# sikoba/babble

Measured on AMD Instinct MI355X. Metric: ECDSA event verifies/sec, higher is better.
Workload: dtype u32; 1 GPU; C2: VerifyBatch of 1M signed Events per GPU (64 creators, 1x64-B tx, ~446-B bodies); per-key tables rebuilt every step; events_per_gpu=1000000, creators=64, parallelism=single, batches_in_flight=2

## Files before the change

### babble_amd/csrc/point.h

```cpp
#pragma once
#include "field.h"

struct gej {
  fe X, Y, Z;
};

DEV void gej_double(gej &r, const gej &a) {
  fe A, B, C, D, E, F, t;
  fe_sqr(A, a.X);
  fe_sqr(B, a.Y);
  fe_sqr(C, B);
  fe_add(t, a.X, B);
  fe_sqr(t, t);
  fe_sub(t, t, A);
  fe_sub(t, t, C);
  fe_dbl(D, t);
  fe_dbl(E, A);
  fe_add(E, E, A);
  fe_sqr(F, E);
  fe Z3;
  fe_mul(Z3, a.Y, a.Z);
  fe_dbl(r.Z, Z3);
  fe_dbl(t, D);
  fe_sub(r.X, F, t);
  fe_sub(t, D, r.X);
  fe_mul(r.Y, E, t);
  fe_dbl(t, C);
  fe_dbl(t, t);
  fe_dbl(t, t);
  fe_sub(r.Y, r.Y, t);
}

DEV void gej_double_lat(gej &r, const gej &a) {
#if defined(__HIP_DEVICE_COMPILE__)
  fe A, B, YZ, C, t, E, F, D;
  fe_sqr_sqr_mul_zip_asm(A, a.X, B, a.Y, YZ, a.Y, a.Z);
  fe_add(t, a.X, B);
  fe_dbl(E, A);
  fe_add(E, E, A);
  fe_sqr_sqr_sqr_zip_asm(C, B, t, t, F, E);
  fe_sub(t, t, A);
  fe_sub(t, t, C);
  fe_dbl(D, t);
  fe_dbl(r.Z, YZ);
  fe_dbl(t, D);
  fe_sub(r.X, F, t);
  fe_sub(t, D, r.X);
  fe_mul(r.Y, E, t);
  fe_dbl(t, C);
  fe_dbl(t, t);
  fe_dbl(t, t);
  fe_sub(r.Y, r.Y, t);
#else
  gej_double(r, a);
#endif
}

DEV void gej_add_ge(gej &r, bool &inf, const fe &x2, const fe &y2) {
  if (inf) {
    r.X = x2;
    r.Y = y2;
    fe_set(r.Z, 1);
    inf = false;
    return;
  }
  fe Z1Z1, U2, S2, H, R, t;
  fe_sqr(Z1Z1, r.Z);
  fe_mul(U2, x2, Z1Z1);
  fe_mul(t, r.Z, Z1Z1);
  fe_mul(S2, y2, t);
  fe_sub(H, U2, r.X);
  fe_sub(R, S2, r.Y);
  if (fe_is_zero(H)) {
    if (fe_is_zero(R)) {
      gej d;
      gej_double(d, r);
      r = d;
    } else {
      inf = true;
    }
    return;
  }
  fe HH, HHH, V;
  fe_sqr(HH, H);
  fe_mul(HHH, H, HH);
  fe_mul(V, r.X, HH);
  fe_mul(r.Z, r.Z, H);
  fe_sqr(t, R);
  fe_sub(t, t, HHH);
  fe_sub(t, t, V);
  fe_sub(r.X, t, V);
  fe_sub(t, V, r.X);
  fe_mul(t, R, t);
  fe_mul(HHH, r.Y, HHH);
  fe_sub(r.Y, t, HHH);
}

DEV void gej_add_ge_lat(gej &r, bool &inf, const fe &x2, const fe &y2) {
#if defined(__HIP_DEVICE_COMPILE__)
  if (inf) {
    r.X = x2;
    r.Y = y2;
    fe_set(r.Z, 1);
    inf = false;
    return;
  }
  fe Z1Z1, U2, S2, H, R, t, HH, HHH, V, Z3, RR;
  fe_sqr(Z1Z1, r.Z);
  fe_mul_mul_zip_asm(U2, x2, Z1Z1, t, r.Z, Z1Z1);
  fe_sub(H, U2, r.X);
  fe_mul_sqr_zip_asm(S2, y2, t, HH, H);
  fe_sub(R, S2, r.Y);
  if (fe_is_zero(H)) {
    if (fe_is_zero(R)) {
      gej d;
      gej_double_lat(d, r);
      r = d;
    } else {
      inf = true;
    }
    return;
  }
  fe_mul_mul_mul_sqr_zip_asm(HHH, H, HH, V, r.X, HH, Z3, r.Z, H, RR, R);
  r.Z = Z3;
  fe_sub(t, RR, HHH);
  fe_sub(t, t, V);
  fe_sub(r.X, t, V);
  fe_sub(t, V, r.X);
  fe_mul_mul_zip_asm(t, R, t, HHH, r.Y, HHH);
  fe_sub(r.Y, t, HHH);
#else
  gej_add_ge(r, inf, x2, y2);
#endif
}

template <bool LAT>
DEV void gej_add_ge_sel(gej &r, bool &inf, const fe &x2, const fe &y2) {
  if (LAT) gej_add_ge_lat(r, inf, x2, y2);
  else gej_add_ge(r, inf, x2, y2);
}
template <bool LAT>
DEV void gej_double_sel(gej &r, const gej &a) {
  if (LAT) gej_double_lat(r, a);
  else gej_double(r, a);
}

DEV void gej_add(gej &r, bool &rinf, const gej &b, bool binf) {
  if (binf) return;
  if (rinf) {
    r = b;
    rinf = false;
    return;
  }
  fe Z1Z1, Z2Z2, U1, U2, S1, S2, H, I, J, rr, V, t;
  fe_sqr(Z1Z1, r.Z);
  fe_sqr(Z2Z2, b.Z);
  fe_mul(U1, r.X, Z2Z2);
  fe_mul(U2, b.X, Z1Z1);
  fe_mul(t, b.Z, Z2Z2);
  fe_mul(S1, r.Y, t);
  fe_mul(t, r.Z, Z1Z1);
  fe_mul(S2, b.Y, t);
  fe_sub(H, U2, U1);
  fe_sub(rr, S2, S1);
  if (fe_is_zero(H)) {
    if (fe_is_zero(rr)) {
      gej d;
      gej_double(d, r);
      r = d;
    } else {
      rinf = true;
    }
    return;
  }
  fe_dbl(I, H);
  fe_sqr(I, I);
  fe_mul(J, H, I);
  fe_dbl(rr, rr);
  fe_mul(V, U1, I);
  fe_add(t, r.Z, b.Z);
  fe_sqr(t, t);
  fe_sub(t, t, Z1Z1);
  fe_sub(t, t, Z2Z2);
  fe_mul(r.Z, t, H);
  fe_sqr(t, rr);
  fe_sub(t, t, J);
  fe_sub(t, t, V);
  fe_sub(r.X, t, V);
  fe_sub(t, V, r.X);
  fe_mul(t, rr, t);
  fe_mul(J, S1, J);
  fe_dbl(J, J);
  fe_sub(r.Y, t, J);
}

struct gexz {
  fe X, Y, ZZ, ZZZ;
};

DEV void gexz_double(gexz &r, const gexz &a) {
  fe U, V, W, S, M, t;
  fe_dbl(U, a.Y);
  fe_sqr(V, U);
  fe_mul(W, U, V);
  fe_mul(S, a.X, V);
  fe_sqr(M, a.X);
  fe_dbl(t, M);
  fe_add(M, M, t);
  fe_sqr(t, M);
  fe_dbl(r.X, S);
  fe_sub(r.X, t, r.X);
  fe_sub(t, S, r.X);
  fe_mul(t, M, t);
  fe_mul(U, W, a.Y);
  fe_sub(r.Y, t, U);
  fe_mul(r.ZZ, V, a.ZZ);
  fe_mul(r.ZZZ, W, a.ZZZ);
}

DEV void gexz_set_ge(gexz &r, const fe &x, const fe &y) {
  r.X = x;
  r.Y = y;
  fe_set(r.ZZ, 1);
  fe_set(r.ZZZ, 1);
}

DEV void gexz_add_ge(gexz &r, bool &inf, const fe &x2, const fe &y2) {
  if (inf) {
    gexz_set_ge(r, x2, y2);
    inf = false;
    return;
  }
  fe P, R, PP, PPP, Q, t;
  fe_mul(P, x2, r.ZZ);
  fe_sub(P, P, r.X);
  fe_mul(R, y2, r.ZZZ);
  fe_sub(R, R, r.Y);
  if (fe_is_zero(P)) {
    if (fe_is_zero(R)) {
      gexz d;
      gexz_double(d, r);
      r = d;
    } else {
      inf = true;
    }
    return;
  }
  fe_sqr(PP, P);
  fe_mul(PPP, P, PP);
  fe_mul(Q, r.X, PP);
  fe_mul(r.ZZ, r.ZZ, PP);
  fe_sqr(t, R);
  fe_sub(t, t, PPP);
  fe_sub(t, t, Q);
  fe_sub(r.X, t, Q);
  fe_sub(t, Q, r.X);
  fe_mul(t, R, t);
  fe_mul(r.ZZZ, r.ZZZ, PPP);
  fe_mul(PPP, r.Y, PPP);
  fe_sub(r.Y, t, PPP);
}

DEV void gexz_add_ge_lat(gexz &r, bool &inf, const fe &x2, const fe &y2) {
#if defined(__HIP_DEVICE_COMPILE__)
  if (inf) {
    gexz_set_ge(r, x2, y2);
    inf = false;
    return;
  }
  fe P, R, PP, RR, PPP, Q, ZZ3, t, u;
  fe_mul_mul_zip_asm(P, x2, r.ZZ, R, y2, r.ZZZ);
  fe_sub(P, P, r.X);
  fe_sub(R, R, r.Y);
  if (fe_is_zero(P)) {
    if (fe_is_zero(R)) {
      gexz d;
      gexz_double(d, r);
      r = d;
    } else {
      inf = true;
    }
    return;
  }
  fe_sqr_sqr_zip_asm(PP, P, RR, R);
  fe_mul_mul_mul_zip_asm(PPP, P, PP, Q, r.X, PP, ZZ3, r.ZZ, PP);
  r.ZZ = ZZ3;
  fe_sub(t, RR, PPP);
  fe_sub(t, t, Q);
  fe_sub(r.X, t, Q);
  fe_sub(t, Q, r.X);
  fe_mul_mul_mul_zip_asm(t, R, t, u, r.Y, PPP, ZZ3, r.ZZZ, PPP);
  r.ZZZ = ZZ3;
  fe_sub(r.Y, t, u);
#else
  gexz_add_ge(r, inf, x2, y2);
#endif
}

DEV void gexz_add(gexz &r, bool &rinf, const gexz &b, bool binf) {
  if (binf) return;
  if (rinf) {
    r = b;
    rinf = false;
    return;
  }
  fe U1, U2, S1, S2, P, R, PP, PPP, Q, t;
  fe_mul(U1, r.X, b.ZZ);
  fe_mul(U2, b.X, r.ZZ);
  fe_mul(S1, r.Y, b.ZZZ);
  fe_mul(S2, b.Y, r.ZZZ);
  fe_sub(P, U2, U1);
  fe_sub(R, S2, S1);
  if (fe_is_zero(P)) {
    if (fe_is_zero(R)) {
      gexz d;
      gexz_double(d, r);
      r = d;
    } else {
      rinf = true;
    }
    return;
  }
  fe_sqr(PP, P);
  fe_mul(PPP, P, PP);
  fe_mul(Q, U1, PP);
  fe_sqr(t, R);
  fe_sub(t, t, PPP);
  fe_sub(t, t, Q);
  fe_sub(r.X, t, Q);
  fe_sub(t, Q, r.X);
  fe_mul(t, R, t);
  fe_mul(S1, S1, PPP);
  fe_sub(r.Y, t, S1);
  fe_mul(r.ZZ, r.ZZ, b.ZZ);
  fe_mul(r.ZZ, r.ZZ, PP);
  fe_mul(r.ZZZ, r.ZZZ, b.ZZZ);
  fe_mul(r.ZZZ, r.ZZZ, PPP);
}

DEV void gexz_add_lat(gexz &r, bool &rinf, const gexz &b, bool binf) {
#if defined(__HIP_DEVICE_COMPILE__)
  if (binf) return;
  if (rinf) {
    r = b;
    rinf = false;
    return;
  }
  fe U1, U2, S1, S2, Z12, W12, P, R, PP, RR, PPP, Q, t, u;
  fe_mul_mul_mul_zip_asm(U1, r.X, b.ZZ, U2, b.X, r.ZZ, S1, r.Y, b.ZZZ);
  fe_mul_mul_mul_zip_asm(S2, b.Y, r.ZZZ, Z12, r.ZZ, b.ZZ, W12, r.ZZZ, b.ZZZ);
  fe_sub(P, U2, U1);
  fe_sub(R, S2, S1);
  if (fe_is_zero(P)) {
    if (fe_is_zero(R)) {
      gexz d;
      gexz_double(d, r);
      r = d;
    } else {
      rinf = true;
    }
    return;
  }
  fe_sqr_sqr_zip_asm(PP, P, RR, R);
  fe_mul_mul_mul_zip_asm(PPP, P, PP, Q, U1, PP, r.ZZ, Z12, PP);
  fe_sub(t, RR, PPP);
  fe_sub(t, t, Q);
  fe_sub(r.X, t, Q);
  fe_sub(t, Q, r.X);
  fe_mul_mul_mul_zip_asm(t, R, t, u, S1, PPP, r.ZZZ, W12, PPP);
  fe_sub(r.Y, t, u);
#else
  gexz_add(r, rinf, b, binf);
#endif
}

DEV void gexz_sum_ge_lat(gexz &r, bool &rinf, const fe &x1, const fe &y1, bool i1, const fe &x2, const fe &y2,
                         bool i2) {
  rinf = i1 && i2;
  if (i1 || i2) {
    if (!rinf) gexz_set_ge(r, i1 ? x2 : x1, i1 ? y2 : y1);
    return;
  }
  fe P, R;
  fe_sub(P, x2, x1);
  fe_sub(R, y2, y1);
  if (fe_is_zero(P)) {
    if (fe_is_zero(R)) {
      gexz a;
      gexz_set_ge(a, x1, y1);
      gexz_double(r, a);
    } else {
      rinf = true;
    }
    return;
  }
#if defined(__HIP_DEVICE_COMPILE__)
  fe PP, RR, PPP, Q, t, u;
  fe_sqr_sqr_zip_asm(PP, P, RR, R);
  fe_mul_mul_zip_asm(PPP, P, PP, Q, x1, PP);
  fe_sub(t, RR, PPP);
  fe_sub(t, t, Q);
  fe_sub(r.X, t, Q);
  fe_sub(t, Q, r.X);
  fe_mul_mul_zip_asm(t, R, t, u, y1, PPP);
  fe_sub(r.Y, t, u);
  r.ZZ = PP;
  r.ZZZ = PPP;
#else
  gexz_set_ge(r, x1, y1);
  gexz_add_ge(r, rinf, x2, y2);
#endif
}

DEV void gexz_from_gej(gexz &r, const gej &a) {
  r.X = a.X;
  r.Y = a.Y;
  fe_sqr(r.ZZ, a.Z);
  fe_mul(r.ZZZ, r.ZZ, a.Z);
}

template <bool LAT>
DEV void pt_add_ge(gexz &r, bool &inf, const fe &x2, const fe &y2) {
  if (LAT) gexz_add_ge_lat(r, inf, x2, y2);
  else gexz_add_ge(r, inf, x2, y2);
}

template <bool LAT>
DEV void gexz_add_ge_aff(gexz &r, bool &inf, const fe &x2, const fe &y2) {
  fe P, R, PP, RR, PPP, Q, t, u, v;
  fe_sub(P, x2, r.X);
  fe_sub(R, y2, r.Y);
  if (fe_is_zero(P)) {
    if (fe_is_zero(R)) {
      gexz d;
      gexz_double(d, r);
      r = d;
    } else {
      inf = true;
    }
    return;
  }
#if defined(__HIP_DEVICE_COMPILE__)
  if (LAT) {
    fe_sqr_sqr_zip_asm(PP, P, RR, R);
    fe_mul_mul_zip_asm(PPP, P, PP, Q, r.X, PP);
  } else
#endif
  {
    fe_sqr(PP, P);
    fe_sqr(RR, R);
    fe_mul(PPP, P, PP);
    fe_mul(Q, r.X, PP);
  }
  fe_sub(t, RR, PPP);
  fe_sub(t, t, Q);
  fe_sub(t, t, Q);
  fe_sub(u, Q, t);
  r.X = t;
  r.ZZ = PP;
  r.ZZZ = PPP;
#if defined(__HIP_DEVICE_COMPILE__)
  if (LAT) {
    fe_mul_mul_zip_asm(t, R, u, v, r.Y, PPP);
  } else
#endif
  {
    fe_mul(t, R, u);
    fe_mul(v, r.Y, PPP);
  }
  fe_sub(r.Y, t, v);
}

template <bool LAT>
DEV void pt_add_ge_step(gexz &r, bool &inf, const fe &x2, const fe &y2, bool take) {
  if (take) pt_add_ge<LAT>(r, inf, x2, y2);
}
template <bool LAT>
DEV void pt_add_ge_step(gej &r, bool &inf, const fe &x2, const fe &y2, bool take) {
  if (take) gej_add_ge_sel<LAT>(r, inf, x2, y2);
}
template <bool LAT>
DEV void pt_add_ge(gej &r, bool &inf, const fe &x2, const fe &y2) {
  gej_add_ge_sel<LAT>(r, inf, x2, y2);
}
```

### babble_amd/csrc/verify_core.h

```cpp
#pragma once
#include <type_traits>
#include <stdint.h>

#include "../../include/babbleverify.h"
#include "geometry.h"
#include "coop.h"
#include "point.h"
#include "sha256.h"

#define KS_OK 0
#define KS_EMPTY 1
#define KS_BAD 2

static constexpr uint32_t P_MINUS_N[8] = {0x2FC9BAEEu, 0x402DA172u, 0x50B75FC4u, 0x45512319u,
                                          0x00000001u, 0u, 0u, 0u};

DEV void fe_load_be(fe &r, const uint8_t *b) {
#pragma unroll
  for (int i = 0; i < 8; i++) {
    const uint8_t *q = b + 4 * (7 - i);
    r.v[i] = ((uint32_t)q[0] << 24) | ((uint32_t)q[1] << 16) | ((uint32_t)q[2] << 8) | q[3];
  }
}
DEV void fe_load_be_words(fe &r, const uint32_t *w) {
#pragma unroll
  for (int i = 0; i < 8; i++) r.v[i] = bswap32(w[7 - i]);
}
DEV void sc_load_be_words(sc &r, const uint32_t *w) {
#pragma unroll
  for (int i = 0; i < 8; i++) r.v[i] = bswap32(w[7 - i]);
}
DEV void fe_store(uint32_t *p, const fe &a) {
#pragma unroll
  for (int i = 0; i < 8; i++) p[i] = a.v[i];
}
DEV void fe_load(fe &a, const uint32_t *p) {
#pragma unroll
  for (int i = 0; i < 8; i++) a.v[i] = p[i];
}
DEV void fe_load4(fe &a, const uint32_t *p) {
#if defined(__HIP_DEVICE_COMPILE__)
  typedef const __attribute__((address_space(1))) uint4 *gptr;
  const gptr q = (gptr)p;
#else
  const uint4 *q = (const uint4 *)p;
#endif
  uint4 l = q[0], h = q[1];
  a.v[0] = l.x; a.v[1] = l.y; a.v[2] = l.z; a.v[3] = l.w;
  a.v[4] = h.x; a.v[5] = h.y; a.v[6] = h.z; a.v[7] = h.w;
}
DEV void store16(uint32_t *p, const uint32_t *v) {
  uint4 *q = (uint4 *)p;
#pragma unroll
  for (int c = 0; c < 4; c++) q[c] = make_uint4(v[4 * c], v[4 * c + 1], v[4 * c + 2], v[4 * c + 3]);
}
DEV bool u256_lt(const uint32_t *a, const uint32_t *b) {
#pragma unroll
  for (int i = 7; i >= 0; i--) {
    if (a[i] != b[i]) return a[i] < b[i];
  }
  return false;
}
DEV bool u256_is_zero(const uint32_t *a) {
  uint32_t x = 0;
#pragma unroll
  for (int i = 0; i < 8; i++) x |= a[i];
  return x == 0;
}

DEV void sha256_one(uint64_t m, const uint8_t *bytes, const uint64_t *off, uint32_t *digest_words) {
  const uint64_t o = off[m];
  const uint64_t len = off[m + 1] - o;
  uint32_t h[8];
  sha256_msg(h, bytes, o, len);
  uint32_t be[8];
#pragma unroll
  for (int i = 0; i < 8; i++) be[i] = bswap32(h[i]);
  uint4 *dst = (uint4 *)(digest_words + 8 * m);
  dst[0] = make_uint4(be[0], be[1], be[2], be[3]);
  dst[1] = make_uint4(be[4], be[5], be[6], be[7]);
}

DEV void key_decode_point(const uint8_t *kbytes, uint64_t o, uint64_t len, uint8_t &st, fe &x, fe &y) {
  st = KS_BAD;
  fe_set(x, 0);
  fe_set(y, 0);
  if (len == 0) {
    st = KS_EMPTY;
  } else if (len == 65 && kbytes[o] == 4) {
#if defined(__HIP_DEVICE_COMPILE__)
    const uint32_t *w = (const uint32_t *)(kbytes + (o & ~(uint64_t)3));
    const uint32_t sh = (uint32_t)(o & 3);
    uint32_t d[18];
#pragma unroll
    for (int i = 0; i < 18; i++) d[i] = w[i];
#pragma unroll
    for (int i = 0; i < 8; i++) {
      const uint32_t bx = 1 + 4 * (7 - i) + sh, by = 33 + 4 * (7 - i) + sh;
      x.v[i] = bswap32(alignbyte(d[bx / 4 + 1], d[bx / 4], bx % 4));
      y.v[i] = bswap32(alignbyte(d[by / 4 + 1], d[by / 4], by % 4));
    }
#else
    fe_load_be(x, kbytes + o + 1);
    fe_load_be(y, kbytes + o + 33);
#endif
    if (!fe_ge_p(x) && !fe_ge_p(y)) {
      fe y2, x3, seven;
      fe_sqr(y2, y);
      fe_sqr(x3, x);
      fe_mul(x3, x3, x);
      fe_set(seven, 7);
      fe_add(x3, x3, seven);
      if (fe_eq(y2, x3)) st = KS_OK;
    }
  }
}

DEV void key_decode_one(uint32_t k, const uint8_t *kbytes, const uint64_t *koff, uint8_t *kstatus, uint32_t *kxy) {
  uint8_t st;
  fe x, y;
  key_decode_point(kbytes, koff[k], koff[k + 1] - koff[k], st, x, y);
  kstatus[k] = st;
  fe_store(kxy + 16 * k, x);
  fe_store(kxy + 16 * k + 8, y);
}

template <bool LAT = false>
DEV void table_bases_one(uint32_t b, const uint32_t *bxy, uint32_t *bases_jac, int w, int nwin) {
  gej P;
  fe_load(P.X, bxy + 16 * b);
  fe_load(P.Y, bxy + 16 * b + 8);
  fe_set(P.Z, 1);
  uint32_t *out = bases_jac + (uint64_t)b * nwin * 24;
  for (int j = 0; j < nwin; j++) {
    fe_store(out + 24 * j, P.X);
    fe_store(out + 24 * j + 8, P.Y);
    fe_store(out + 24 * j + 16, P.Z);
    if (j + 1 < nwin) {
      for (int k = 0; k < w; k++) gej_double_sel<LAT>(P, P);
    }
  }
}

#if defined(__HIPCC__)
__device__ __forceinline__ void coop_bases_one(uint32_t b, const uint32_t *bxy, uint32_t *bases_jac, int w, int nwin) {
  const uint32_t k = coop::pos(), lane = __lane_id();
  uint32_t X = k < 8 ? bxy[16 * (uint64_t)b + k] : 0u, Y = k < 8 ? bxy[16 * (uint64_t)b + 8 + k] : 0u;
  uint32_t Z = k == 0 ? 1u : 0u;
  uint32_t *out = bases_jac + (uint64_t)b * nwin * 24;
  for (int j = 0; j < nwin; j++) {
    if (lane < 8) {
      out[24 * j + lane] = X;
      out[24 * j + 8 + lane] = Y;
      out[24 * j + 16 + lane] = Z;
    }
    if (j + 1 < nwin)
      for (int i = 0; i < w; i++) coop::dbl(X, Y, Z);
  }
}
#endif

template <bool LAT = false>
DEV void table_point(gej &R, bool &inf, fe &Z, const fe &bx, const fe &by, uint32_t d, int bits) {
  inf = true;
  fe_set(R.X, 0);
  fe_set(R.Y, 0);
  fe_set(R.Z, 0);
  for (int bit = bits - 1; bit >= 0; bit--) {
    if (!inf) gej_double_sel<LAT>(R, R);
    if ((d >> bit) & 1) gej_add_ge_sel<LAT>(R, inf, bx, by);
  }
  if (inf) fe_set(Z, 1);
  else Z = R.Z;
}

DEV void table_store(uint32_t *entry, uint32_t *phi, uint32_t d, const gej &R, bool inf, const fe &zi) {
  fe zi2, zi3, x, y;
  fe_sqr(zi2, zi);
  fe_mul(zi3, zi2, zi);
  fe_mul(x, R.X, zi2);
  fe_mul(y, R.Y, zi3);
  fe_canon(x);
  fe_canon(y);
  if (d == 0 || inf) {
    fe_set(x, 0);
    fe_set(y, 0);
  }
  uint32_t v[16];
#pragma unroll
  for (int i = 0; i < 8; i++) {
    v[i] = x.v[i];
    v[8 + i] = y.v[i];
  }
  store16(entry, v);
  if (phi) {
    fe beta, bx;
    fe_load(beta, FE_BETA);
    fe_mul(bx, x, beta);
    fe_canon(bx);
#pragma unroll
    for (int i = 0; i < 8; i++) v[i] = bx.v[i];
    store16(phi, v);
  }
}

DEV int pair_kind(uint32_t lo, uint32_t hi) { return (lo ? 1 : 0) | (hi ? 2 : 0); }

DEV uint32_t k12_digit(uint32_t d, uint32_t ent) { return d ? d : ent; }

DEV void pair_load(const uint32_t *s_lo, const uint32_t *s_hi, uint32_t lo, uint32_t hi, fe &x1, fe &y1, fe &x2,
                   fe &y2) {
  fe_load(x1, s_lo + BV_ENTRY_U32 * lo);
  fe_load(y1, s_lo + BV_ENTRY_U32 * lo + 8);
  fe_load(x2, s_hi + BV_ENTRY_U32 * hi);
  fe_load(y2, s_hi + BV_ENTRY_U32 * hi + 8);
}

DEV void pair_denominator(fe &H, int kind, const fe &x1, const fe &x2) {
  if (kind == 3) fe_sub(H, x2, x1);
  else fe_set(H, 1);
}

DEV void pair_store(uint32_t *entry, uint32_t *phi, int kind, const fe &x1, const fe &y1, const fe &x2, const fe &y2,
                    const fe &Hinv) {
  fe x, y;
  if (kind == 3) {
    fe lam, t;
    fe_sub(t, y2, y1);
    fe_mul(lam, t, Hinv);
    fe_sqr(x, lam);
    fe_sub(x, x, x1);
    fe_sub(x, x, x2);
    fe_sub(t, x1, x);
    fe_mul(y, lam, t);
    fe_sub(y, y, y1);
  } else if (kind == 1) {
    x = x1;
    y = y1;
  } else {
    x = x2;
    y = y2;
  }
  fe_canon(x);
  fe_canon(y);
  uint32_t v[16];
#pragma unroll
  for (int i = 0; i < 8; i++) {
    v[i] = x.v[i];
    v[8 + i] = y.v[i];
  }
  store16(entry, v);
  if (!phi) return;
  fe beta, bx;
  fe_load(beta, FE_BETA);
  fe_mul(bx, x, beta);
  fe_canon(bx);
#pragma unroll
  for (int i = 0; i < 8; i++) v[i] = bx.v[i];
  store16(phi, v);
}

DEV void sc_sqrn(sc &a, int n) {
#pragma unroll 1
  for (int i = 0; i < n; i++) sc_mont(a, a, a);
}

DEV void sc_inverse(sc &r, const sc &x) {
  sc x2, x3, x5, x7, x9, x11, x13, x15;
  sc_mont(x2, x, x);
  sc_mont(x3, x2, x);
  sc_mont(x5, x3, x2);
  sc_mont(x7, x5, x2);
  sc_mont(x9, x7, x2);
  sc_mont(x11, x9, x2);
  sc_mont(x13, x11, x2);
  sc_mont(x15, x13, x2);
  sc a2 = x3, a4, a8, a16, a32, a64, t;
  a4 = a2; sc_sqrn(a4, 2); sc_mont(a4, a4, a2);
  a8 = a4; sc_sqrn(a8, 4); sc_mont(a8, a8, a4);
  a16 = a8; sc_sqrn(a16, 8); sc_mont(a16, a16, a8);
  a32 = a16; sc_sqrn(a32, 16); sc_mont(a32, a32, a16);
  a64 = a32; sc_sqrn(a64, 32); sc_mont(a64, a64, a32);
  t = a64;
  sc_sqrn(t, 32); sc_mont(t, t, a32);
  sc_sqrn(t, 16); sc_mont(t, t, a16);
  sc_sqrn(t, 8); sc_mont(t, t, a8);
  sc_sqrn(t, 4); sc_mont(t, t, a4);
  sc_sqrn(t, 2); sc_mont(t, t, a2);
  sc_sqrn(t, 1); sc_mont(t, t, x);
  sc_sqrn(t, 1);
#define SQM(n, m) sc_sqrn(t, n); sc_mont(t, t, m);
  SQM(4, x11) SQM(3, x5) SQM(4, x5) SQM(4, x7) SQM(5, x13) SQM(2, x3) SQM(5, x7) SQM(6, x13)
  SQM(5, x11) SQM(4, x13) SQM(3, x) SQM(6, x5) SQM(10, x7) SQM(4, x7) SQM(5, x15) SQM(4, x15)
  SQM(5, x9) SQM(6, x11) SQM(4, x13) SQM(5, x3) SQM(6, x13) SQM(10, x13) SQM(4, x9) SQM(9, x9)
  SQM(4, x15) SQM(1, x)
#undef SQM
  r = t;
}

DEV bool s_usable(const uint8_t *pre, uint64_t i, const sc &s) {
  return (pre == nullptr || pre[i] == 0) && !u256_is_zero(s.v) && u256_lt(s.v, SC_N);
}

DEV void sinv_thread(uint64_t t, uint64_t T, uint64_t n_items, uint32_t M, const uint32_t *s_be, const uint8_t *pre,
                     uint32_t *w_out) {
  sc R1, one;
  sc_load_const(R1, SC_R1);
#pragma unroll
  for (int k = 0; k < 8; k++) one.v[k] = k == 0 ? 1u : 0u;
  sc acc = R1;
  for (uint32_t m = 0; m < M; m++) {
    const uint64_t i = t + (uint64_t)m * T;
    if (i >= n_items) break;
    sc s;
    sc_load_be_words(s, s_be + 8 * i);
    if (!s_usable(pre, i, s)) s = one;
    uint4 *q = (uint4 *)(w_out + 8 * i);
    q[0] = make_uint4(acc.v[0], acc.v[1], acc.v[2], acc.v[3]);
    q[1] = make_uint4(acc.v[4], acc.v[5], acc.v[6], acc.v[7]);
    sc_mont(acc, acc, s);
  }
  sc inv;
  sc_inverse_var(inv, acc);
  sc_mont(inv, inv, one);
  for (int m = (int)M - 1; m >= 0; m--) {
    const uint64_t i = t + (uint64_t)m * T;
    if (i >= n_items) continue;
    sc s, pfx, w;
    sc_load_be_words(s, s_be + 8 * i);
    if (!s_usable(pre, i, s)) s = one;
    uint4 *q = (uint4 *)(w_out + 8 * i);
    const uint4 a = q[0], b = q[1];
    pfx.v[0] = a.x; pfx.v[1] = a.y; pfx.v[2] = a.z; pfx.v[3] = a.w;
    pfx.v[4] = b.x; pfx.v[5] = b.y; pfx.v[6] = b.z; pfx.v[7] = b.w;
    sc_mont(w, inv, pfx);
    sc_mont(inv, inv, s);
    q[0] = make_uint4(w.v[0], w.v[1], w.v[2], w.v[3]);
    q[1] = make_uint4(w.v[4], w.v[5], w.v[6], w.v[7]);
  }
}

DEV void item_scalars(uint64_t i, const uint32_t *r_be, const uint32_t *item_msg, const uint32_t *digest_words,
                      const uint32_t *w_in, uint32_t u1[8], uint32_t k1[4], uint32_t k2[4], uint32_t &signs) {
  sc w, e, r, a, b;
  const uint4 *q = (const uint4 *)(w_in + 8 * i);
  const uint4 x = q[0], y = q[1];
  w.v[0] = x.x; w.v[1] = x.y; w.v[2] = x.z; w.v[3] = x.w;
  w.v[4] = y.x; w.v[5] = y.y; w.v[6] = y.z; w.v[7] = y.w;
  sc_load_be_words(e, digest_words + 8 * (uint64_t)item_msg[i]);
  sc_load_be_words(r, r_be + 8 * i);
  sc_mont(a, e, w);
  sc_mont(b, r, w);
#pragma unroll
  for (int k = 0; k < 8; k++) u1[k] = a.v[k];
  glv_split(k1, k2, signs, b);
}

#define BV_DEFERRED 0xFE

DEV uint8_t classify(uint8_t pre, uint8_t ks, const fe &r, const fe &s) {
  if (pre & BV_PRE_PARTS_BAD) return BV_REJECT_ERR;
  if (ks == KS_EMPTY) return BV_REF_PANIC;
  uint32_t rc = pre & 3u, scl = (pre >> 2) & 3u;
  if (rc == BV_SC_OK) rc = u256_is_zero(r.v) ? BV_SC_NONPOS : (u256_lt(r.v, SC_N) ? BV_SC_OK : BV_SC_GE_N);
  if (scl == BV_SC_OK) scl = u256_is_zero(s.v) ? BV_SC_NONPOS : (u256_lt(s.v, SC_N) ? BV_SC_OK : BV_SC_GE_N);
  if (rc == BV_SC_NIL) return BV_REF_PANIC;
  if (rc == BV_SC_NONPOS) return BV_REJECT;
  if (scl == BV_SC_NIL) return BV_REF_PANIC;
  if (scl == BV_SC_NONPOS) return BV_REJECT;
  if (rc == BV_SC_GE_N || scl == BV_SC_GE_N) return BV_REJECT;
  if (ks != KS_OK) return BV_REF_PANIC;
  return 0xFF;
}

DEV uint8_t classify_item(uint64_t i, const uint32_t *item_key, const uint32_t *r_be, const uint32_t *s_be,
                          const uint8_t *pre, const uint8_t *kstatus, fe &r) {
  fe s;
  fe_load_be_words(r, r_be + 8 * i);
  fe_load_be_words(s, s_be + 8 * i);
  return classify(pre ? pre[i] : 0, kstatus[item_key[i]], r, s);
}

DEV bool final_check(const gej &R, bool inf, const fe &r) {
  if (inf) return false;
  fe z2, t;
  fe_sqr(z2, R.Z);
  fe_mul(t, r, z2);
  if (fe_eq(t, R.X)) return true;
  if (u256_lt(r.v, P_MINUS_N)) {
    fe rn;
    uint32_t c = 0;
#pragma unroll
    for (int i = 0; i < 8; i++) rn.v[i] = addc32(r.v[i], SC_N[i], c);
    fe_mul(t, rn, z2);
    if (fe_eq(t, R.X)) return true;
  }
  return false;
}

DEV bool final_check(const gexz &R, bool inf, const fe &r) {
  if (inf) return false;
  fe t;
  fe_mul(t, r, R.ZZ);
  if (fe_eq(t, R.X)) return true;
  if (u256_lt(r.v, P_MINUS_N)) {
    fe rn;
    uint32_t c = 0;
#pragma unroll
    for (int i = 0; i < 8; i++) rn.v[i] = addc32(r.v[i], SC_N[i], c);
    fe_mul(t, rn, R.ZZ);
    if (fe_eq(t, R.X)) return true;
  }
  return false;
}

template <int W, int NWIN, bool LAT = false, class PT = gej, bool FROM_INF = false>
DEV void g_table_add(PT &R, bool &inf, const uint32_t *tab, uint32_t u[8]) {
  constexpr uint32_t ENT = 1u << (W - 1);
  static_assert(W * NWIN >= 257 && W < 32, "signed G windows must absorb the last carry");
  uint32_t carry = 0;
  for (int j = 0; j < NWIN; j++) {
    uint32_t d = (u[0] & ((1u << W) - 1u)) + carry;
#pragma unroll
    for (int c = 0; c < 7; c++) u[c] = (u[c] >> W) | (u[c + 1] << (32 - W));
    u[7] >>= W;
    carry = d > ENT ? 1u : 0u;
    const bool dneg = carry != 0;
    if (dneg) d = (1u << W) - d;
    const uint32_t *e = tab + ((uint64_t)j * ENT + d) * BV_ENTRY_U32;
    fe x, y;
    fe_load4(x, e);
    fe_load4(y, e + 8);
    fe_cneg_canon(y, dneg);
    if constexpr (FROM_INF) {
      if (j == 1 && !inf) {
        if (d != 0) gexz_add_ge_aff<LAT>(R, inf, x, y);
        continue;
      }
    }
    pt_add_ge_step<LAT>(R, inf, x, y, d != 0);
  }
}

DEV void load_k(uint32_t k1[4], uint32_t k2[4], uint32_t &signs, const uint32_t *u12, uint64_t i) {
  const uint4 *q = (const uint4 *)(u12 + (uint64_t)BV_U_STRIDE * i);
  uint4 a = q[0], b = q[1], c = q[2];
  k1[0] = a.x; k1[1] = a.y; k1[2] = a.z; k1[3] = a.w;
  k2[0] = b.x; k2[1] = b.y; k2[2] = b.z; k2[3] = b.w;
  signs = c.x;
}

#define RG_WORDS 33
DEV void rg_store(uint32_t *rg, uint64_t n, uint64_t i, const gexz &R, bool inf) {
#pragma unroll
  for (int k = 0; k < 8; k++) {
    rg[(uint64_t)k * n + i] = R.X.v[k];
    rg[(uint64_t)(8 + k) * n + i] = R.Y.v[k];
    rg[(uint64_t)(16 + k) * n + i] = R.ZZ.v[k];
    rg[(uint64_t)(24 + k) * n + i] = R.ZZZ.v[k];
  }
  rg[(uint64_t)32 * n + i] = inf ? 1u : 0u;
}
DEV void rg_load(const uint32_t *rg, uint64_t n, uint64_t i, gexz &R, bool &inf) {
#pragma unroll
  for (int k = 0; k < 8; k++) {
    R.X.v[k] = rg[(uint64_t)k * n + i];
    R.Y.v[k] = rg[(uint64_t)(8 + k) * n + i];
    R.ZZ.v[k] = rg[(uint64_t)(16 + k) * n + i];
    R.ZZZ.v[k] = rg[(uint64_t)(24 + k) * n + i];
  }
  inf = rg[(uint64_t)32 * n + i] != 0;
}

DEV void glv_split_item(uint64_t i, const uint32_t *r_be, const uint32_t *w_in, uint32_t *u12) {
  sc w, r, b;
  const uint4 *q = (const uint4 *)(w_in + 8 * i);
  const uint4 x = q[0], y = q[1];
  w.v[0] = x.x; w.v[1] = x.y; w.v[2] = x.z; w.v[3] = x.w;
  w.v[4] = y.x; w.v[5] = y.y; w.v[6] = y.z; w.v[7] = y.w;
  sc_load_be_words(r, r_be + 8 * i);
  sc_mont(b, r, w);
  uint32_t k1[4], k2[4], signs;
  glv_split(k1, k2, signs, b);
  uint4 *o = (uint4 *)(u12 + (uint64_t)BV_U_STRIDE * i);
  o[0] = make_uint4(k1[0], k1[1], k1[2], k1[3]);
  o[1] = make_uint4(k2[0], k2[1], k2[2], k2[3]);
  o[2] = make_uint4(signs, 0u, 0u, 0u);
}

template <bool LAT = false, bool SPLIT = false>
DEV void verify_item_g(uint64_t i, uint64_t n, const uint32_t *item_key, const uint32_t *r_be, const uint32_t *s_be,
                       const uint8_t *pre, const uint8_t *kstatus, const uint32_t *item_msg,
                       const uint32_t *digest_words, const uint32_t *w_in, uint32_t *u12, const uint32_t *g_table,
                       uint32_t *rg) {
  fe r;
  if (classify_item(i, item_key, r_be, s_be, pre, kstatus, r) != 0xFF) return;
  uint32_t u[8];
  if (SPLIT) {
    sc w, e, a;
    const uint4 *q = (const uint4 *)(w_in + 8 * i);
    const uint4 x = q[0], y = q[1];
    w.v[0] = x.x; w.v[1] = x.y; w.v[2] = x.z; w.v[3] = x.w;
    w.v[4] = y.x; w.v[5] = y.y; w.v[6] = y.z; w.v[7] = y.w;
    sc_load_be_words(e, digest_words + 8 * (uint64_t)item_msg[i]);
    sc_mont(a, e, w);
#pragma unroll
    for (int k = 0; k < 8; k++) u[k] = a.v[k];
  } else {
    uint32_t k1[4], k2[4], signs;
    item_scalars(i, r_be, item_msg, digest_words, w_in, u, k1, k2, signs);
    uint4 *q = (uint4 *)(u12 + (uint64_t)BV_U_STRIDE * i);
    q[0] = make_uint4(k1[0], k1[1], k1[2], k1[3]);
    q[1] = make_uint4(k2[0], k2[1], k2[2], k2[3]);
    q[2] = make_uint4(signs, 0u, 0u, 0u);
  }
  gexz R;
  bool inf = true;
  fe_set(R.X, 0);
  fe_set(R.Y, 0);
  fe_set(R.ZZ, 0);
  fe_set(R.ZZZ, 0);
  g_table_add<BV_GW, BV_GNWIN, LAT, gexz, true>(R, inf, g_table, u);
  rg_store(rg, n, i, R, inf);
}

template <int W, int NWIN, bool SIGNED, bool LAT = false, class PT = gexz>
DEV void key_table_add(PT &R, bool &inf, const uint32_t *tab, uint32_t k[4], bool neg, bool phi = false,
                       bool from_inf = false) {
  constexpr uint32_t ENT = SIGNED ? (1u << (W - 1)) : (1u << W);
  static_assert(!SIGNED || W * NWIN >= 129, "signed windows must absorb the last carry");
  if (neg) fe_neg(R.Y, R.Y);
  uint32_t carry = 0;
  for (int j = 0; j < NWIN; j++) {
    uint32_t d = (k[0] & ((1u << W) - 1u)) + carry;
    k[0] = (k[0] >> W) | (k[1] << (32 - W));
    k[1] = (k[1] >> W) | (k[2] << (32 - W));
    k[2] = (k[2] >> W) | (k[3] << (32 - W));
    k[3] >>= W;
    bool dneg = false;
    if (SIGNED) {
      carry = d > ENT ? 1u : 0u;
      if (carry) {
        d = (1u << W) - d;
        dneg = true;
      }
    }
    const uint32_t *e = tab + ((uint64_t)j * ENT + d) * BV_ENTRY_U32;
    fe x, y;
    fe_load4(x, e);
    fe_load4(y, e + 8);
    if (phi) {
      fe beta;
      fe_load(beta, FE_BETA);
      fe_mul(x, x, beta);
    }
    fe_cneg_canon(y, dneg);
    if constexpr (std::is_same<PT, gexz>::value) {
      if (from_inf && j == 1 && !inf) {
        if (d != 0) gexz_add_ge_aff<LAT>(R, inf, x, y);
        continue;
      }
    }
    pt_add_ge_step<LAT>(R, inf, x, y, d != 0);
  }
  if (neg) fe_neg(R.Y, R.Y);
}

template <int W, int NWIN, bool LAT = false>
DEV uint8_t verify_item_q(uint64_t i, uint64_t n, const uint32_t *item_key, const uint32_t *r_be,
                          const uint32_t *s_be, const uint8_t *pre, const uint8_t *kstatus, const uint32_t *u12,
                          const uint32_t *key_table, const uint64_t *key_tabs, const uint32_t *rg) {
  constexpr bool SIGNED = W != BV_KW;
  constexpr bool KC = W == BV_KCW;
  constexpr uint64_t half =
      SIGNED ? ((uint64_t)NWIN * (1ull << (W - 1)) + 1) * BV_ENTRY_U32 : (uint64_t)NWIN * (1ull << W) * BV_ENTRY_U32;
  static_assert(W != BV_K12W || half == BV_K12HALF_U32, "K12 geometry");
  static_assert(!KC || half == BV_KCHALF_U32, "KC geometry");
  fe r;
  const uint8_t st = classify_item(i, item_key, r_be, s_be, pre, kstatus, r);
  if (st != 0xFF) return st;
  uint32_t k1[4], k2[4], signs;
  load_k(k1, k2, signs, u12, i);
  gexz R;
  bool inf;
  rg_load(rg, n, i, R, inf);
  const uint32_t *tab = key_tabs ? (const uint32_t *)key_tabs[item_key[i]]
                                 : key_table + (uint64_t)item_key[i] * (KC ? 1 : 2) * half;
  if (!tab) return BV_DEFERRED;
#pragma unroll 1
  for (int h = 0; h < 2; h++) {
    uint32_t kk[4];
#pragma unroll
    for (int c = 0; c < 4; c++) kk[c] = h ? k2[c] : k1[c];
    key_table_add<W, NWIN, SIGNED, LAT>(R, inf, tab + (h && !KC ? half : 0), kk, (signs >> h) & 1u, KC && h);
  }
  fe_load_be_words(r, r_be + 8 * i);
  return final_check(R, inf, r) ? BV_ACCEPT : BV_REJECT;
}

template <int W, int NWIN, bool LAT = false>
DEV void verify_item_qfirst(uint64_t i, uint64_t n, const uint32_t *item_key, const uint32_t *r_be,
                            const uint32_t *s_be, const uint8_t *pre, const uint8_t *kstatus, const uint32_t *w_in,
                            const uint32_t *key_table, const uint64_t *key_tabs, uint32_t *rq) {
  constexpr bool SIGNED = W != BV_KW;
  constexpr bool KC = W == BV_KCW;
  constexpr uint64_t half =
      SIGNED ? ((uint64_t)NWIN * (1ull << (W - 1)) + 1) * BV_ENTRY_U32 : (uint64_t)NWIN * (1ull << W) * BV_ENTRY_U32;
  fe r;
  if (classify_item(i, item_key, r_be, s_be, pre, kstatus, r) != 0xFF) return;
  uint32_t k1[4], k2[4], signs;
  {
    sc w, rs, b;
    const uint4 *q = (const uint4 *)(w_in + 8 * i);
    const uint4 x = q[0], y = q[1];
    w.v[0] = x.x; w.v[1] = x.y; w.v[2] = x.z; w.v[3] = x.w;
    w.v[4] = y.x; w.v[5] = y.y; w.v[6] = y.z; w.v[7] = y.w;
    sc_load_be_words(rs, r_be + 8 * i);
    sc_mont(b, rs, w);
    glv_split(k1, k2, signs, b);
  }
  gexz R;
  bool inf = true;
  fe_set(R.X, 0);
  fe_set(R.Y, 0);
  fe_set(R.ZZ, 0);
  fe_set(R.ZZZ, 0);
  const uint32_t *tab = key_tabs ? (const uint32_t *)key_tabs[item_key[i]]
                                 : key_table + (uint64_t)item_key[i] * (KC ? 1 : 2) * half;
  if (!tab) {
    rq[(uint64_t)32 * n + i] = 2u;
    return;
  }
#pragma unroll 1
  for (int h = 0; h < 2; h++) {
    uint32_t kk[4];
#pragma unroll
    for (int c = 0; c < 4; c++) kk[c] = h ? k2[c] : k1[c];
    key_table_add<W, NWIN, SIGNED, LAT>(R, inf, tab + (h && !KC ? half : 0), kk, (signs >> h) & 1u, KC && h,
                                        h == 0);
  }
  rg_store(rq, n, i, R, inf);
}

template <bool LAT = false>
DEV uint8_t verify_item_gfinish(uint64_t i, uint64_t n, const uint32_t *item_key, const uint32_t *r_be,
                                const uint32_t *s_be, const uint8_t *pre, const uint8_t *kstatus,
                                const uint32_t *item_msg, const uint32_t *digest_words, const uint32_t *w_in,
                                const uint32_t *g_table, const uint32_t *rq) {
  fe r;
  const uint8_t st = classify_item(i, item_key, r_be, s_be, pre, kstatus, r);
  if (st != 0xFF) return st;
  if (rq[(uint64_t)32 * n + i] == 2u) return BV_DEFERRED;
  uint32_t u[8];
  {
    sc w, e, a;
    const uint4 *q = (const uint4 *)(w_in + 8 * i);
    const uint4 x = q[0], y = q[1];
    w.v[0] = x.x; w.v[1] = x.y; w.v[2] = x.z; w.v[3] = x.w;
    w.v[4] = y.x; w.v[5] = y.y; w.v[6] = y.z; w.v[7] = y.w;
    sc_load_be_words(e, digest_words + 8 * (uint64_t)item_msg[i]);
    sc_mont(a, e, w);
#pragma unroll
    for (int k = 0; k < 8; k++) u[k] = a.v[k];
  }
  gexz R;
  bool inf;
  rg_load(rq, n, i, R, inf);
  g_table_add<BV_GW, BV_GNWIN, LAT>(R, inf, g_table, u);
  fe_load_be_words(r, r_be + 8 * i);
  return final_check(R, inf, r) ? BV_ACCEPT : BV_REJECT;
}

template <bool LAT = false>
DEV uint8_t verify_item_gq_kc(uint64_t i, const uint32_t *item_key, const uint32_t *r_be, const uint32_t *s_be,
                              const uint8_t *pre, const uint8_t *kstatus, const uint32_t *item_msg,
                              const uint32_t *digest_words, const uint32_t *w_in, const uint32_t *g_table,
                              const uint64_t *key_tabs) {
  fe r;
  const uint8_t st = classify_item(i, item_key, r_be, s_be, pre, kstatus, r);
  if (st != 0xFF) return st;
  const uint32_t *tab = (const uint32_t *)key_tabs[item_key[i]];
  if (!tab) return BV_DEFERRED;
  uint32_t u[8], k1[4], k2[4], signs;
  item_scalars(i, r_be, item_msg, digest_words, w_in, u, k1, k2, signs);
  gexz R;
  bool inf = true;
  fe_set(R.X, 0);
  fe_set(R.Y, 0);
  fe_set(R.ZZ, 0);
  fe_set(R.ZZZ, 0);
  g_table_add<BV_GW, BV_GNWIN, LAT, gexz, true>(R, inf, g_table, u);
#pragma unroll 1
  for (int h = 0; h < 2; h++) {
    uint32_t kk[4];
#pragma unroll
    for (int c = 0; c < 4; c++) kk[c] = h ? k2[c] : k1[c];
    key_table_add<BV_KCW, BV_KCNWIN, true, LAT>(R, inf, tab, kk, (signs >> h) & 1u, h != 0);
  }
  fe_load_be_words(r, r_be + 8 * i);
  return final_check(R, inf, r) ? BV_ACCEPT : BV_REJECT;
}

template <bool LAT = false>
DEV uint8_t verify_item_generic(uint64_t i, const uint32_t *item_key, const uint32_t *r_be, const uint32_t *s_be,
                                const uint8_t *pre, const uint8_t *kstatus, const uint32_t *kxy,
                                const uint32_t *item_msg, const uint32_t *digest_words, const uint32_t *w_in,
                                const uint32_t *g_table) {
  fe r;
  const uint8_t st = classify_item(i, item_key, r_be, s_be, pre, kstatus, r);
  if (st != 0xFF) return st;
  const uint32_t k = item_key[i];
  uint32_t u1[8], k1[4], k2[4], signs;
  item_scalars(i, r_be, item_msg, digest_words, w_in, u1, k1, k2, signs);
  fe q1x, q1y, q2x, q2y, beta;
  fe_load(q1x, kxy + 16 * k);
  fe_load(q1y, kxy + 16 * k + 8);
  fe_load(beta, FE_BETA);
  fe_mul(q2x, q1x, beta);
  q2y = q1y;
  if (signs & 1u) fe_neg(q1y, q1y);
  if (signs & 2u) fe_neg(q2y, q2y);
  gej R;
  bool inf = true;
  fe_set(R.X, 0);
  fe_set(R.Y, 0);
  fe_set(R.Z, 0);
  for (int bit = 127; bit >= 0; bit--) {
    if (!inf) gej_double_sel<LAT>(R, R);
    if ((k1[bit >> 5] >> (bit & 31)) & 1u) gej_add_ge_sel<LAT>(R, inf, q1x, q1y);
    if ((k2[bit >> 5] >> (bit & 31)) & 1u) gej_add_ge_sel<LAT>(R, inf, q2x, q2y);
  }
  g_table_add<BV_GW, BV_GNWIN, LAT>(R, inf, g_table, u1);
  return final_check(R, inf, r) ? BV_ACCEPT : BV_REJECT;
}

DEV void sinv_one(sc &w, const sc &s) {
  sc t, one;
#pragma unroll
  for (int k = 0; k < 8; k++) one.v[k] = k == 0 ? 1u : 0u;
  sc_inverse_var(t, s);
  sc_mont(w, t, one);
}

DEV void scalars_from(const sc &w, const sc &e, const sc &r, uint32_t u1[8], uint32_t k1[4], uint32_t k2[4],
                      uint32_t &signs) {
  sc a, b;
  sc_mont(a, e, w);
  sc_mont(b, r, w);
#pragma unroll
  for (int k = 0; k < 8; k++) u1[k] = a.v[k];
  glv_split(k1, k2, signs, b);
}

template <int W, int NWIN, bool LAT = false, class PT = gexz>
DEV void g_table_add_range(PT &R, bool &inf, const uint32_t *tab, uint32_t u[8], int j0, int j1) {
  constexpr uint32_t ENT = 1u << (W - 1);
  uint32_t carry = 0;
  for (int j = 0; j < NWIN; j++) {
    uint32_t d = (u[0] & ((1u << W) - 1u)) + carry;
#pragma unroll
    for (int c = 0; c < 7; c++) u[c] = (u[c] >> W) | (u[c + 1] << (32 - W));
    u[7] >>= W;
    carry = d > ENT ? 1u : 0u;
    const bool dneg = carry != 0;
    if (dneg) d = (1u << W) - d;
    if (j < j0 || j >= j1) continue;
    const uint32_t *e = tab + ((uint64_t)j * ENT + d) * BV_ENTRY_U32;
    fe x, y;
    fe_load4(x, e);
    fe_load4(y, e + 8);
    fe_cneg_canon(y, dneg);
    pt_add_ge_step<LAT>(R, inf, x, y, d != 0);
  }
}

template <bool LAT = false>
DEV void naf_mul(gej &R, bool &inf, const fe &px, const fe &py, const uint32_t k[4]) {
  uint32_t h[5], kk[5], pos[5], neg[5];
  uint32_t c = 0;
#pragma unroll
  for (int i = 0; i < 4; i++) kk[i] = k[i];
  kk[4] = 0;
  uint32_t prev = 0;
#pragma unroll
  for (int i = 0; i < 5; i++) {
    const uint32_t k2 = (kk[i] << 1) | (prev >> 31);
    prev = kk[i];
    h[i] = addc32(kk[i], k2, c);
  }
#pragma unroll
  for (int i = 0; i < 5; i++) {
    const uint32_t x = h[i] ^ kk[i];
    pos[i] = x & h[i];
    neg[i] = x & kk[i];
  }
#pragma unroll
  for (int i = 0; i < 5; i++) {
    pos[i] = (pos[i] >> 1) | (i < 4 ? pos[i + 1] << 31 : 0u);
    neg[i] = (neg[i] >> 1) | (i < 4 ? neg[i + 1] << 31 : 0u);
  }
  fe ny;
  fe_neg(ny, py);
  inf = true;
  fe_set(R.X, 0);
  fe_set(R.Y, 0);
  fe_set(R.Z, 0);
  for (int bit = 129; bit >= 0; bit--) {
    if (!inf) gej_double_sel<LAT>(R, R);
    const uint32_t p = (pos[bit >> 5] >> (bit & 31)) & 1u, n = (neg[bit >> 5] >> (bit & 31)) & 1u;
    if (p | n) gej_add_ge_sel<LAT>(R, inf, px, n ? ny : py);
  }
}

template <int W, int NW>
DEV void table_leaf(fe &x, fe &y, bool &zero, const uint32_t *tab, uint32_t u[NW], int j, bool neg, bool phi) {
  constexpr uint32_t ENT = 1u << (W - 1);
  uint32_t carry = 0, d = 0;
  for (int w = 0; w <= j; w++) {
    d = (u[0] & ((1u << W) - 1u)) + carry;
#pragma unroll
    for (int c = 0; c < NW - 1; c++) u[c] = (u[c] >> W) | (u[c + 1] << (32 - W));
    u[NW - 1] >>= W;
    carry = d > ENT ? 1u : 0u;
  }
  const bool dneg = carry != 0;
  if (dneg) d = (1u << W) - d;
  zero = d == 0;
  const uint32_t *e = tab + ((uint64_t)j * ENT + d) * BV_ENTRY_U32;
  fe_load4(x, e);
  fe_load4(y, e + 8);
  if (phi) {
    fe beta;
    fe_load(beta, FE_BETA);
    fe_mul(x, x, beta);
  }
  fe_cneg_canon(y, dneg != neg);
}

DEV void part_store(uint32_t *p, const gexz &R, bool inf) {
#pragma unroll
  for (int k = 0; k < 8; k++) p[k] = R.X.v[k], p[8 + k] = R.Y.v[k], p[16 + k] = R.ZZ.v[k], p[24 + k] = R.ZZZ.v[k];
  p[32] = inf ? 1u : 0u;
}
DEV void part_load(const uint32_t *p, gexz &R, bool &inf) {
#pragma unroll
  for (int k = 0; k < 8; k++) R.X.v[k] = p[k], R.Y.v[k] = p[8 + k], R.ZZ.v[k] = p[16 + k], R.ZZZ.v[k] = p[24 + k];
  inf = p[32] != 0;
}
```

Measured before the change: 512.9 million verifies/s.

## Prefetch table entries into LDS one window ahead via async global_load_lds

Table lookups in the G and per-key window loops are now software-pipelined: the next window's entry is issued as an asynchronous global-to-LDS load while the current point addition runs, and then read back from shared memory. The aim is to hide global memory latency behind field arithmetic. The change also folds the GLV sign negation into the per-entry conditional negate, skips the Y/ZZZ update on the final addition since the final check only needs X and ZZ, and parks k2 in LDS to lower register pressure. In exchange it uses extra LDS per block, hardcodes 256-lane staging slots with wave-level indexing, and only applies to the non-LAT gexz path.

```diff
diff --git a/babble_amd/csrc/point.h b/babble_amd/csrc/point.h
--- a/babble_amd/csrc/point.h
+++ b/babble_amd/csrc/point.h
@@ -225,7 +225,7 @@
   fe_set(r.ZZZ, 1);
 }
 
-DEV void gexz_add_ge(gexz &r, bool &inf, const fe &x2, const fe &y2) {
+DEV void gexz_add_ge(gexz &r, bool &inf, const fe &x2, const fe &y2, bool xz_only = false) {
   if (inf) {
     gexz_set_ge(r, x2, y2);
     inf = false;
@@ -254,6 +254,7 @@
   fe_sub(t, t, PPP);
   fe_sub(t, t, Q);
   fe_sub(r.X, t, Q);
+  if (xz_only) return;
   fe_sub(t, Q, r.X);
   fe_mul(t, R, t);
   fe_mul(r.ZZZ, r.ZZZ, PPP);
@@ -420,9 +421,9 @@
 }
 
 template <bool LAT>
-DEV void pt_add_ge(gexz &r, bool &inf, const fe &x2, const fe &y2) {
+DEV void pt_add_ge(gexz &r, bool &inf, const fe &x2, const fe &y2, bool xz_only = false) {
   if (LAT) gexz_add_ge_lat(r, inf, x2, y2);
-  else gexz_add_ge(r, inf, x2, y2);
+  else gexz_add_ge(r, inf, x2, y2, xz_only);
 }
 
 template <bool LAT>
@@ -472,11 +473,11 @@
 }
 
 template <bool LAT>
-DEV void pt_add_ge_step(gexz &r, bool &inf, const fe &x2, const fe &y2, bool take) {
-  if (take) pt_add_ge<LAT>(r, inf, x2, y2);
-}
-template <bool LAT>
-DEV void pt_add_ge_step(gej &r, bool &inf, const fe &x2, const fe &y2, bool take) {
+DEV void pt_add_ge_step(gexz &r, bool &inf, const fe &x2, const fe &y2, bool take, bool xz_only = false) {
+  if (take) pt_add_ge<LAT>(r, inf, x2, y2, xz_only);
+}
+template <bool LAT>
+DEV void pt_add_ge_step(gej &r, bool &inf, const fe &x2, const fe &y2, bool take, bool xz_only = false) {
   if (take) gej_add_ge_sel<LAT>(r, inf, x2, y2);
 }
 template <bool LAT>
diff --git a/babble_amd/csrc/verify_core.h b/babble_amd/csrc/verify_core.h
--- a/babble_amd/csrc/verify_core.h
+++ b/babble_amd/csrc/verify_core.h
@@ -414,11 +414,133 @@
   return false;
 }
 
-template <int W, int NWIN, bool LAT = false, class PT = gej, bool FROM_INF = false>
+#ifndef BV_LOOKUP_PIPE
+#define BV_LOOKUP_PIPE 3
+#endif
+#define BV_STAGE_LANES 256
+
+#if defined(__HIP_DEVICE_COMPILE__)
+__device__ __forceinline__ uint4 *entry_stage_slots() {
+  __shared__ uint4 slots[4 * BV_STAGE_LANES];
+  return slots;
+}
+#endif
+
+struct entry_stage {
+#if defined(__HIP_DEVICE_COMPILE__)
+  DEV void request(const uint32_t *e) {
+    typedef __attribute__((address_space(1))) uint4 *gptr;
+    typedef __attribute__((address_space(3))) uint4 *lptr;
+    asm volatile("s_waitcnt lgkmcnt(0)" ::: "memory");
+    const gptr g = (gptr)e;
+    const lptr w = (lptr)entry_stage_slots() + __builtin_amdgcn_readfirstlane(threadIdx.x & ~63u);
+#pragma unroll
+    for (int c = 0; c < 4; c++)
+      __builtin_amdgcn_global_load_lds((__attribute__((address_space(1))) void *)(g + c),
+                                       (__attribute__((address_space(3))) void *)(w + c * BV_STAGE_LANES), 16, 0, 0);
+  }
+  DEV void take(fe &x, fe &y) {
+    asm volatile("s_waitcnt vmcnt(0)" ::: "memory");
+    const uint4 *s = entry_stage_slots() + threadIdx.x;
+    const uint4 a = s[0], b = s[BV_STAGE_LANES], c = s[2 * BV_STAGE_LANES], d = s[3 * BV_STAGE_LANES];
+    x.v[0] = a.x; x.v[1] = a.y; x.v[2] = a.z; x.v[3] = a.w;
+    x.v[4] = b.x; x.v[5] = b.y; x.v[6] = b.z; x.v[7] = b.w;
+    y.v[0] = c.x; y.v[1] = c.y; y.v[2] = c.z; y.v[3] = c.w;
+    y.v[4] = d.x; y.v[5] = d.y; y.v[6] = d.z; y.v[7] = d.w;
+  }
+#else
+  uint32_t buf[BV_ENTRY_U32];
+  DEV void request(const uint32_t *e) {
+    for (int k = 0; k < BV_ENTRY_U32; k++) buf[k] = e[k];
+  }
+  DEV void take(fe &x, fe &y) {
+    for (int k = 0; k < 8; k++) x.v[k] = buf[k], y.v[k] = buf[8 + k];
+  }
+#endif
+};
+
+struct lane_park {
+#if defined(__HIP_DEVICE_COMPILE__)
+  DEV uint4 *slot() {
+    __shared__ uint4 park[BV_STAGE_LANES];
+    return park + threadIdx.x;
+  }
+  DEV void put(const uint32_t v[4]) { *slot() = make_uint4(v[0], v[1], v[2], v[3]); }
+  DEV void get(uint32_t v[4]) {
+    const uint4 a = *slot();
+    v[0] = a.x; v[1] = a.y; v[2] = a.z; v[3] = a.w;
+  }
+#else
+  uint32_t buf[4];
+  DEV void put(const uint32_t v[4]) {
+    for (int c = 0; c < 4; c++) buf[c] = v[c];
+  }
+  DEV void get(uint32_t v[4]) {
+    for (int c = 0; c < 4; c++) v[c] = buf[c];
+  }
+#endif
+};
+
+template <bool PARK>
+DEV void glv_half(uint32_t kk[4], int h, const uint32_t k1[4], const uint32_t k2[4], lane_park &park) {
+  if (PARK) {
+    if (h) park.get(kk);
+    else
+#pragma unroll
+      for (int c = 0; c < 4; c++) kk[c] = k1[c];
+  } else {
+#pragma unroll
+    for (int c = 0; c < 4; c++) kk[c] = h ? k2[c] : k1[c];
+  }
+}
+
+template <int W, int NL, bool SIGNED>
+DEV uint32_t next_digit(uint32_t *u, uint32_t &carry, bool &dneg) {
+  constexpr uint32_t ENT = 1u << (W - 1);
+  uint32_t d = (u[0] & ((1u << W) - 1u)) + carry;
+#pragma unroll
+  for (int c = 0; c < NL - 1; c++) u[c] = (u[c] >> W) | (u[c + 1] << (32 - W));
+  u[NL - 1] >>= W;
+  dneg = false;
+  if (SIGNED) {
+    carry = d > ENT ? 1u : 0u;
+    dneg = carry != 0;
+    if (dneg) d = (1u << W) - d;
+  }
+  return d;
+}
+
+template <int W, int NWIN, bool LAT = false, class PT = gej, bool FROM_INF = false, bool FINAL = false>
 DEV void g_table_add(PT &R, bool &inf, const uint32_t *tab, uint32_t u[8]) {
   constexpr uint32_t ENT = 1u << (W - 1);
   static_assert(W * NWIN >= 257 && W < 32, "signed G windows must absorb the last carry");
   uint32_t carry = 0;
+  if constexpr ((BV_LOOKUP_PIPE & 1) && !LAT && std::is_same<PT, gexz>::value) {
+    entry_stage stage;
+    bool dneg;
+    uint32_t d = next_digit<W, 8, true>(u, carry, dneg);
+    stage.request(tab + (uint64_t)d * BV_ENTRY_U32);
+#pragma unroll 1
+    for (int j = 0; j < NWIN; j++) {
+      fe x, y;
+      stage.take(x, y);
+      const uint32_t dj = d;
+      const bool nj = dneg;
+      if (j + 1 < NWIN) {
+        d = next_digit<W, 8, true>(u, carry, dneg);
+        stage.request(tab + ((uint64_t)(j + 1) * ENT + d) * BV_ENTRY_U32);
+      }
+      fe_cneg_canon(y, nj);
+      if constexpr (FROM_INF) {
+        if (j == 1 && !inf) {
+          if (dj != 0) gexz_add_ge_aff<LAT>(R, inf, x, y);
+          continue;
+        }
+      }
+      pt_add_ge_step<LAT>(R, inf, x, y, dj != 0, FINAL && j == NWIN - 1);
+    }
+    return;
+  }
   for (int j = 0; j < NWIN; j++) {
     uint32_t d = (u[0] & ((1u << W) - 1u)) + carry;
 #pragma unroll
@@ -438,7 +560,7 @@
         continue;
       }
     }
-    pt_add_ge_step<LAT>(R, inf, x, y, d != 0);
+    pt_add_ge_step<LAT>(R, inf, x, y, d != 0, FINAL && j == NWIN - 1);
   }
 }
 
@@ -526,11 +648,41 @@
 
 template <int W, int NWIN, bool SIGNED, bool LAT = false, class PT = gexz>
 DEV void key_table_add(PT &R, bool &inf, const uint32_t *tab, uint32_t k[4], bool neg, bool phi = false,
-                       bool from_inf = false) {
+                       bool from_inf = false, bool last = false) {
   constexpr uint32_t ENT = SIGNED ? (1u << (W - 1)) : (1u << W);
   static_assert(!SIGNED || W * NWIN >= 129, "signed windows must absorb the last carry");
-  if (neg) fe_neg(R.Y, R.Y);
   uint32_t carry = 0;
+  if constexpr ((BV_LOOKUP_PIPE & 2) && !LAT && std::is_same<PT, gexz>::value) {
+    entry_stage stage;
+    bool dneg;
+    uint32_t d = next_digit<W, 4, SIGNED>(k, carry, dneg);
+    stage.request(tab + (uint64_t)d * BV_ENTRY_U32);
+#pragma unroll 1
+    for (int j = 0; j < NWIN; j++) {
+      fe x, y;
+      stage.take(x, y);
+      const uint32_t dj = d;
+      const bool nj = dneg != neg;
+      if (j + 1 < NWIN) {
+        d = next_digit<W, 4, SIGNED>(k, carry, dneg);
+        stage.request(tab + ((uint64_t)(j + 1) * ENT + d) * BV_ENTRY_U32);
+      }
+      if (phi) {
+        fe beta;
+        fe_load(beta, FE_BETA);
+        fe_mul(x, x, beta);
+      }
+      fe_cneg_canon(y, nj);
+      if (from_inf && j == 1 && !inf) {
+        if (dj != 0) gexz_add_ge_aff<LAT>(R, inf, x, y);
+        continue;
+      }
+      pt_add_ge_step<LAT>(R, inf, x, y, dj != 0, last && j == NWIN - 1);
+    }
+    return;
+  }
+  constexpr bool fold = !LAT;
+  if (!fold && neg) fe_neg(R.Y, R.Y);
   for (int j = 0; j < NWIN; j++) {
     uint32_t d = (k[0] & ((1u << W) - 1u)) + carry;
     k[0] = (k[0] >> W) | (k[1] << (32 - W));
@@ -554,16 +706,16 @@
       fe_load(beta, FE_BETA);
       fe_mul(x, x, beta);
     }
-    fe_cneg_canon(y, dneg);
+    fe_cneg_canon(y, dneg != (fold && neg));
     if constexpr (std::is_same<PT, gexz>::value) {
       if (from_inf && j == 1 && !inf) {
         if (d != 0) gexz_add_ge_aff<LAT>(R, inf, x, y);
         continue;
       }
     }
-    pt_add_ge_step<LAT>(R, inf, x, y, d != 0);
-  }
-  if (neg) fe_neg(R.Y, R.Y);
+    pt_add_ge_step<LAT>(R, inf, x, y, d != 0, last && j == NWIN - 1);
+  }
+  if (!fold && neg) fe_neg(R.Y, R.Y);
 }
 
 template <int W, int NWIN, bool LAT = false>
@@ -587,12 +739,15 @@
   const uint32_t *tab = key_tabs ? (const uint32_t *)key_tabs[item_key[i]]
                                  : key_table + (uint64_t)item_key[i] * (KC ? 1 : 2) * half;
   if (!tab) return BV_DEFERRED;
+  constexpr bool PARK = (BV_LOOKUP_PIPE & 2) && !LAT;
+  lane_park park;
+  if (PARK) park.put(k2);
 #pragma unroll 1
   for (int h = 0; h < 2; h++) {
     uint32_t kk[4];
-#pragma unroll
-    for (int c = 0; c < 4; c++) kk[c] = h ? k2[c] : k1[c];
-    key_table_add<W, NWIN, SIGNED, LAT>(R, inf, tab + (h && !KC ? half : 0), kk, (signs >> h) & 1u, KC && h);
+    glv_half<PARK>(kk, h, k1, k2, park);
+    key_table_add<W, NWIN, SIGNED, LAT>(R, inf, tab + (h && !KC ? half : 0), kk, (signs >> h) & 1u, KC && h, false,
+                                        h == 1);
   }
   fe_load_be_words(r, r_be + 8 * i);
   return final_check(R, inf, r) ? BV_ACCEPT : BV_REJECT;
@@ -631,11 +786,13 @@
     rq[(uint64_t)32 * n + i] = 2u;
     return;
   }
+  constexpr bool PARK = (BV_LOOKUP_PIPE & 2) && !LAT;
+  lane_park park;
+  if (PARK) park.put(k2);
 #pragma unroll 1
   for (int h = 0; h < 2; h++) {
     uint32_t kk[4];
-#pragma unroll
-    for (int c = 0; c < 4; c++) kk[c] = h ? k2[c] : k1[c];
+    glv_half<PARK>(kk, h, k1, k2, park);
     key_table_add<W, NWIN, SIGNED, LAT>(R, inf, tab + (h && !KC ? half : 0), kk, (signs >> h) & 1u, KC && h,
                                         h == 0);
   }
@@ -666,7 +823,7 @@
   gexz R;
   bool inf;
   rg_load(rq, n, i, R, inf);
-  g_table_add<BV_GW, BV_GNWIN, LAT>(R, inf, g_table, u);
+  g_table_add<BV_GW, BV_GNWIN, LAT, gexz, false, true>(R, inf, g_table, u);
   fe_load_be_words(r, r_be + 8 * i);
   return final_check(R, inf, r) ? BV_ACCEPT : BV_REJECT;
 }
@@ -690,12 +847,14 @@
   fe_set(R.ZZ, 0);
   fe_set(R.ZZZ, 0);
   g_table_add<BV_GW, BV_GNWIN, LAT, gexz, true>(R, inf, g_table, u);
+  constexpr bool PARK = (BV_LOOKUP_PIPE & 2) && !LAT;
+  lane_park park;
+  if (PARK) park.put(k2);
 #pragma unroll 1
   for (int h = 0; h < 2; h++) {
     uint32_t kk[4];
-#pragma unroll
-    for (int c = 0; c < 4; c++) kk[c] = h ? k2[c] : k1[c];
-    key_table_add<BV_KCW, BV_KCNWIN, true, LAT>(R, inf, tab, kk, (signs >> h) & 1u, h != 0);
+    glv_half<PARK>(kk, h, k1, k2, park);
+    key_table_add<BV_KCW, BV_KCNWIN, true, LAT>(R, inf, tab, kk, (signs >> h) & 1u, h != 0, false, h == 1);
   }
   fe_load_be_words(r, r_be + 8 * i);
   return final_check(R, inf, r) ? BV_ACCEPT : BV_REJECT;
```

After: 524.4 million verifies/s (median of 6 runs). +2.2%, better.
